# bioinfologics/w2rap-contigger

Hardware: AMD Instinct MI355X
Metric: step2_k60_canonical_kmers_per_s (higher is better)
Workload: dtype u64

## Files before the change

w2rap_contigger_amd/csrc/ctx.h:

```cpp
#pragma once
#include <hip/hip_runtime.h>
#include <stdint.h>
#include <stdio.h>
#include <stdlib.h>
#include <cstdlib>
#include <string>
#include <utility>
#include <vector>
#include "../../include/w2rap_step2.h"
#include "common.h"

namespace w2 {

struct Ctx;
}
struct w2rap_step2_ctx;
namespace w2 {
struct Ctx {
    int device = 0;
    hipStream_t stream = nullptr;
    hipStream_t stream2 = nullptr;
    unsigned long long* h_pinned = nullptr;
    std::string err;
    int sm_count = 256;

    uint64_t n = 0;
    const uint8_t* d_bases = nullptr;
    const uint64_t* d_boff = nullptr;
    const uint32_t* d_len = nullptr;
    const uint8_t* d_quals = nullptr;
    const uint64_t* d_qoff = nullptr;
    uint32_t max_len = 0;
    std::vector<void*> owned_reads;

    uint16_t* d_good = nullptr;
    uint32_t min_qual = 7, min_freq = 4;

    uint64_t M = 0, D = 0, S = 0;
    uint64_t hist[101] = {0};
    uint32_t NB = 0;
    uint32_t* d_bcount = nullptr;
    unsigned long long part_kmers[64] = {0};
    uint64_t* d_bbase = nullptr;
    uint32_t* d_recs = nullptr;
    uint64_t nrec = 0;
    uint64_t solid_cap = 0;
    uint64_t* d_shi = nullptr;
    uint64_t* d_slo = nullptr;
    uint32_t* d_scc = nullptr;
    Slot* d_table = nullptr;
    uint64_t tcap = 0;
    unsigned long long* d_filter32 = nullptr;
    uint64_t f32words = 0;
    uint8_t* d_sctx = nullptr;
    void* d_nbr = nullptr;
    bool wide_ids = false;
    uint64_t* d_chunk_start = nullptr;
    uint32_t* d_chunk_cnt = nullptr;
    uint64_t nchunks = 0;
    KRec* d_srec = nullptr;
    bool use_index = false;
    uint4* d_index = nullptr;
    uint64_t index_cap = 0, index_entries = 0;
    uint4* d_xindex = nullptr; uint64_t xindex_cap = 0, xindex_kmers = 0;
    bool index_prebuilt = false, bits_ready = false, filter_prebuilt = false;
    unsigned cs_ns = 0;
    unsigned cs_planned = 0;
    uint32_t cs_nbl = 0, cs_nseg = 0; const uint32_t* cs_recs = nullptr;
    bool cs_short_first = false;
    hipEvent_t cs_ev[16] = {};
    unsigned long long* cs_cnt = nullptr;
    uint64_t* cs_off = nullptr;
    uint32_t cs_chunk_cap = 0;
    uint8_t* d_unres = nullptr;
    bool fused_prune = false;
    std::vector<std::pair<uint64_t, uint64_t>> unfused_chunks;
    uint32_t* cs_defer = nullptr;
    uint64_t* g_hi = nullptr; uint64_t* g_lo = nullptr; uint32_t* g_cc = nullptr;
    uint64_t* g_cstart = nullptr; uint32_t* g_ccnt = nullptr;
    uint64_t g_cap = 0, g_n = 0, g_ccap = 0, g_nc = 0;
    bool g_open = false;
    hipEvent_t g_copied = nullptr;
    bool quality_done = false, counted = false, graphed = false, pathed_done = false;
    bool table_built = false;

    uint64_t E = 0;
    uint64_t rank_ends = 0;
    uint32_t* d_edge_nk = nullptr;
    uint64_t* d_edge_off = nullptr;
    uint8_t* d_edge_codes = nullptr;
    uint8_t* d_edge_bits = nullptr;
    uint64_t edge_bases = 0;
    uint64_t NO = 0, NV = 0;
    int32_t* d_fwdX = nullptr;
    int32_t* d_revX = nullptr;
    uint32_t* d_obj_edge = nullptr;
    ObjRec* d_otab = nullptr;
    int32_t* d_left = nullptr;
    int32_t* d_right = nullptr;
    uint64_t* d_from_off = nullptr;
    int32_t* d_from_v = nullptr;
    int32_t* d_from_e = nullptr;
    uint64_t* d_to_off = nullptr;
    int32_t* d_to_v = nullptr;
    int32_t* d_to_e = nullptr;
    int32_t* d_path_offset = nullptr;
    uint64_t* d_path_off = nullptr;
    int32_t* d_path_edges = nullptr;
    uint64_t path_total = 0;
    uint64_t n_pathed = 0, n_multipathed = 0;
    float ms_count = 0, ms_graph = 0, ms_path = 0;

    uint64_t ld_done = 0;
    void* shard = nullptr;
    std::vector<void*> owned;
    void* pump = nullptr;
    const uint32_t* d_qmask = nullptr;
    int qmask_min_qual = -1;
    int hint_min_qual = -1;
    bool hint_graph_only = false;
    bool quals_absent = false;
    uint8_t* d_qring = nullptr;
    void* pump2 = nullptr;
    hipStream_t copy_stream = nullptr;
    void* quals_job = nullptr;
    void* mask_job = nullptr; void* h_mask = nullptr; size_t h_mask_bytes = 0;
    uint32_t n_passes = 0;
// ... 254 lines not shown
```

w2rap_contigger_amd/csrc/step2_count.hip:

```cpp
#include <algorithm>
#include <chrono>
#include <cstdlib>
#include <cstring>
#include <type_traits>
#include "ctx.h"

namespace w2 {

constexpr unsigned QSLOTS = 256;
template <bool MASK>
__global__ void __launch_bounds__(256) k_good_len(uint64_t n, const uint8_t* __restrict__ quals, const uint32_t* __restrict__ qmask,
                                                   const uint64_t* __restrict__ qoff, const uint32_t* __restrict__ len,
                                                   uint32_t min_qual, uint16_t* __restrict__ good,
                                                   unsigned long long* __restrict__ total_kmers,
                                                   uint32_t* __restrict__ max_len) {
    constexpr unsigned CH = 4096;
    __shared__ __attribute__((aligned(16))) uint16_t gbits[CH + 16];
    __shared__ unsigned long long s_sum[4];
    __shared__ uint32_t s_max[4];
    const uint64_t r0 = (uint64_t)blockIdx.x * blockDim.x;
    const uint64_t r = r0 + threadIdx.x;
    const uint64_t rend = r0 + blockDim.x < n ? r0 + blockDim.x : n;
    const uint64_t base0 = qoff[r0], endo = qoff[rend];
    const unsigned shift = MASK ? (unsigned)(base0 & 31) : (unsigned)((reinterpret_cast<uintptr_t>(quals) + base0) & 15);
// ... 2232 lines not shown
}
int local_dict_slice(Ctx& c, uint64_t n_solid, uint64_t expected_total) {
    if (!c.stream2) return 0;
    if (!c.table_built) {
        if (c.d_table) { c.release(c.d_table); c.d_table = nullptr; }
        W2_TRY(table_alloc(c, std::max<uint64_t>(expected_total, n_solid), c.stream2));
        c.table_built = true; c.ld_done = 0;
    }
    if (n_solid > c.solid_cap) n_solid = c.solid_cap;
    if (n_solid > c.ld_done && 10 * c.tcap >= 13 * n_solid) {
        LAUNCH_ON(c, c.stream2, "k_table_insert", k_table_insert, dim3((unsigned)((n_solid - c.ld_done + 255) / 256)), dim3(256), 0, c.ld_done, n_solid,
                  c.d_shi, c.d_slo, c.d_table, c.tcap - 1);
        W2_HIP(hipGetLastError());
        c.ld_done = n_solid;
    }
    return 0;
}
int prune_local_chunks64(Ctx& c, uint8_t* sctx, uint64_t* nbr, uint8_t* unres) {
    hipStream_t st = c.stream;
    W2_HIP(hipMemsetAsync(unres, 0xFF, c.S, st));
    W2_HIP(hipMemsetAsync(sctx, 0xFF, c.S, st));
    if (!c.nchunks || getenv("W2RAP_NO_LOCAL_PRUNE")) return 0;
    const unsigned gl = (unsigned)std::min<uint64_t>(c.nchunks, (uint64_t)c.sm_count * 64);
    PL_LAUNCH(c, uint64_t, gl, c.S, c.nchunks, c.d_chunk_start, c.d_chunk_cnt, c.d_shi, c.d_slo, c.d_scc, sctx, nbr, unres);
    W2_HIP(hipGetLastError());
    return 0;
}
int prune_local_chunks32(Ctx& c, uint8_t* sctx, uint32_t* nbr, uint8_t* unres) {
    hipStream_t st = c.stream;
    W2_HIP(hipMemsetAsync(unres, 0xFF, c.S, st));
    W2_HIP(hipMemsetAsync(sctx, 0xFF, c.S, st));
    if (!c.nchunks || getenv("W2RAP_NO_LOCAL_PRUNE")) return 0;
    const unsigned gl = (unsigned)std::min<uint64_t>(c.nchunks, (uint64_t)c.sm_count * 64);
    PL_LAUNCH(c, uint32_t, gl, c.S, c.nchunks, c.d_chunk_start, c.d_chunk_cnt, c.d_shi, c.d_slo, c.d_scc, sctx, nbr, unres);
    W2_HIP(hipGetLastError());
    return 0;
}

template <class Id>
static int count_table_t(Ctx& c) {
    hipStream_t st = c.stream;
    if (!c.table_built) W2_TRY(table_alloc(c, c.S, st));
    const bool fused = c.fused_prune && sizeof(Id) == 4 && c.d_sctx && c.d_nbr && c.d_unres;
    Id* nbr = nullptr;
    if (fused) nbr = reinterpret_cast<Id*>(c.d_nbr);
    else {
        for (void* p : {(void*)c.d_sctx, (void*)c.d_nbr, (void*)c.d_unres}) if (p) c.release(p);
        c.d_unres = nullptr;
        W2_ALLOC(c.d_sctx, uint8_t, c.S);
        W2_ALLOC(nbr, Id, 2 * c.S);
        c.d_nbr = nbr;
    }
    c.fused_prune = false;
    if (c.S) {
        unsigned g = (unsigned)((c.S + 255) / 256);
        if (!c.table_built) {
            LAUNCH(c, "k_table_insert", k_table_insert, dim3(g), dim3(256), 0, (uint64_t)0, c.S, c.d_shi, c.d_slo, c.d_table, c.tcap - 1);
            W2_HIP(hipGetLastError());
        }
        uint8_t* d_unres = nullptr;
        if (fused) {
            d_unres = c.d_unres; c.d_unres = nullptr;
            for (auto& rg : c.unfused_chunks) {
                const uint64_t nch = rg.second - rg.first;
                if (!nch) continue;
                const unsigned gl = (unsigned)std::min<uint64_t>(nch, (uint64_t)c.sm_count * 64);
                PL_LAUNCH(c, Id, gl, c.S, nch, c.d_chunk_start + rg.first, c.d_chunk_cnt + rg.first, c.d_shi, c.d_slo, c.d_scc, c.d_sctx, nbr, d_unres);
                W2_HIP(hipGetLastError());
            }
        } else if (c.nchunks) {
            W2_ALLOC(d_unres, uint8_t, c.S);
            W2_HIP(hipMemsetAsync(d_unres, 0xFF, c.S, st));
            W2_HIP(hipMemsetAsync(c.d_sctx, 0xFF, c.S, st));
            const unsigned gl = (unsigned)std::min<uint64_t>(c.nchunks, (uint64_t)c.sm_count * 64);
            PL_LAUNCH(c, Id, gl, c.S, c.nchunks, c.d_chunk_start, c.d_chunk_cnt, c.d_shi, c.d_slo, c.d_scc, c.d_sctx, nbr, d_unres);
            W2_HIP(hipGetLastError());
        }
        if (c.table_built && c.stream2) {
            hipEvent_t ev;
            W2_HIP(hipEventCreateWithFlags(&ev, hipEventDisableTiming));
            W2_HIP(hipEventRecord(ev, c.stream2));
            W2_HIP(hipStreamWaitEvent(st, ev, 0));
            (void)hipEventDestroy(ev);
        }
        LAUNCH(c, "k_prune", k_prune<Id>, dim3(g), dim3(256), 0, (uint64_t)0, c.S, c.d_shi, c.d_slo, c.d_scc, c.d_table, c.tcap - 1, c.d_sctx, nbr,
               (const uint8_t*)d_unres);
        W2_HIP(hipGetLastError());
        W2_HIP(hipStreamSynchronize(st));
        if (d_unres) c.release(d_unres);
    }
    W2_HIP(hipStreamSynchronize(st));
    if (c.stream2) W2_HIP(hipStreamSynchronize(c.stream2));
    c.table_built = false;
    c.counted = true;
    return 0;
}
int count_table(Ctx& c) {
    if (c.S >= MAX_SOLID_KMERS) { c.err = "more than 2^32 solid k-mers on one GPU"; return W2RAP_E_LIMIT; }
    const char* wv = getenv("W2RAP_WIDE_IDS");
    c.wide_ids = c.S >= (1ull << 31) - 1 || (wv && atoi(wv) != 0);
    return c.wide_ids ? count_table_t<uint64_t>(c) : count_table_t<uint32_t>(c);
}

static unsigned auto_passes(uint64_t M) {
    size_t free_b = 0, total_b = 0;
    if (hipMemGetInfo(&free_b, &total_b) != hipSuccess || !free_b) return 1;
    const double need = (double)M / 15.0 * REC_BYTES * 1.25;
    unsigned p = (unsigned)(need / ((double)free_b / 4.0)) + 1;
    return std::min(p, 64u);
}

int phase_count(Ctx& c, uint32_t min_qual, uint32_t min_freq) {
    const bool trace = getenv("W2RAP_TRACE") != nullptr;
    auto now = [] { return std::chrono::duration<double>(std::chrono::steady_clock::now().time_since_epoch()).count(); };
    double t0 = now();
    W2_TRY(count_quality(c, min_qual));
    double t1 = now();
    const char* bv = getenv("W2RAP_BATCHES");
    const char* pv = getenv("W2RAP_PASSES");
    unsigned P = pv ? (unsigned)atoi(pv) : c.n_passes;
    if (!P) P = auto_passes(c.M);
    const uint32_t NB = default_buckets(c.M, 1);
    if (P > NB) P = NB;
    if (P < 1) P = 1;
    c.npass = P;
    double t_part = 0, t_cnt = 0;
    for (unsigned p = 0; p < P; ++p) {
        const uint32_t lo = (uint32_t)((uint64_t)NB * p / P), hi = (uint32_t)((uint64_t)NB * (p + 1) / P);
        unsigned nseg = 1;
        c.pass = p;
        double a = now();
        W2_TRY(count_partition_batched(c, NB, bv ? (unsigned)atoi(bv) : 4, &nseg, lo, hi));
        double b = now();
        W2_TRY(count_buckets(c, min_freq, hi - lo, nseg, c.d_recs, c.d_bcount, c.M, P == 1));
        c.release(c.d_recs); c.d_recs = nullptr;
        t_part += b - a; t_cnt += now() - b;
    }
    c.pass = 0; c.npass = 1;
    double t3 = now();
    W2_TRY(count_table(c));
    double t4 = now();
    if (trace) fprintf(stderr, "[w2rap] count: quality %.1f ms, partition %.1f ms, buckets %.1f ms, table %.1f ms (%u pass%s)\n",
                       (t1 - t0) * 1e3, t_part * 1e3, t_cnt * 1e3, (t4 - t3) * 1e3, P, P == 1 ? "" : "es");
    return 0;
}

}
```

w2rap_contigger_amd/csrc/step2_graph.hip:

```cpp
#include <algorithm>
#include "ctx.h"

namespace w2 {

enum { GE_LOOKUP = 1, GE_OFFSET = 2, GE_HINT_MISS = 4, GE_HINT_DUP = 8, GE_ASSIGN = 16, GE_HINT_LEN = 32 };

template <class Id>
__device__ inline Kmer oriented(const uint64_t* shi, const uint64_t* slo, Id v) {
    Kmer k{shi[v >> 1], slo[v >> 1]};
    return (v & 1) ? kmer_rc(k) : k;
}

template <class Id>
__global__ void __launch_bounds__(256) k_links(uint64_t S, const uint64_t* __restrict__ shi, const uint64_t* __restrict__ slo,
                                                const uint8_t* __restrict__ sctx, Id* nbr_nxt0) {
    constexpr Id NONE = NodeId<Id>::NONE, PAL = NodeId<Id>::PAL;
    uint64_t i = (uint64_t)blockIdx.x * blockDim.x + threadIdx.x;
    if (i >= S) return;
    Kmer k{shi[i], slo[i]};
    Id n0 = NONE, n1 = NONE;
    if (!kmer_is_pal(k)) {
        const Id s = nbr_nxt0[2 * i], p = nbr_nxt0[2 * i + 1];
        if (s < PAL) {
            unsigned cj = sctx[s >> 1]; if (s & 1) cj = brev8(cj);
            if (popc4(cj >> 4) == 1) n0 = s;
        }
        if (p < PAL) {
            unsigned cj = sctx[p >> 1]; if (p & 1) cj = brev8(cj);
            if (popc4(cj & 15) == 1) n1 = p ^ (Id)1;
        }
    }
    nbr_nxt0[2 * i] = n0; nbr_nxt0[2 * i + 1] = n1;
}

constexpr unsigned RT_BUF = 3072;
template <class Id>
__global__ void __launch_bounds__(256) k_rank_tiles(uint64_t S, uint64_t nchunks, const uint64_t* __restrict__ cstart,
                                                     const uint32_t* __restrict__ ccnt, const Id* __restrict__ nxt0,
                                                     unsigned long long* __restrict__ w, uint32_t* __restrict__ own,
                                                     Id* __restrict__ spl, unsigned long long* __restrict__ counters, uint64_t spl_cap) {
    constexpr Id NONE = NodeId<Id>::NONE;
    __shared__ __attribute__((aligned(16))) Id s_nx[RT_NODES];
    __shared__ uint32_t s_w[RT_NODES];
    __shared__ Id s_buf[RT_BUF];
    __shared__ uint32_t s_nbuf, s_run;
    __shared__ unsigned long long s_base;
    const unsigned tid = threadIdx.x, lane = tid & 63;
    if (tid == 0) { s_nbuf = 0; s_run = 0; }
    unsigned long long covered = 0;
    uint32_t ends = 0;
    auto flush = [&]() {
        const uint32_t n = s_nbuf;
        if (tid == 0) s_base = n ? atomicAdd(&counters[0], (unsigned long long)n) : 0ull;
        __syncthreads();
        const unsigned long long gb = s_base;
        for (unsigned i = tid; i < n; i += 256) if (gb + i < spl_cap) spl[gb + i] = s_buf[i];
        __syncthreads();
        if (tid == 0) s_nbuf = 0;
        __syncthreads();
    };
    const uint64_t ntiles = cstart ? nchunks : (S + RT - 1) / RT;
    for (uint64_t ch = blockIdx.x; ch < ntiles; ch += gridDim.x) {
        uint64_t c_start; uint32_t c_cnt;
        if (cstart) { c_start = cstart[ch]; c_cnt = ccnt[ch]; if (c_start + c_cnt > S) c_cnt = 0; }
        else { c_start = ch * RT; c_cnt = (uint32_t)(S - c_start < RT ? S - c_start : RT); }
        covered += c_cnt;
        for (uint32_t sub = 0; sub < c_cnt; sub += RT) {
            const uint64_t base = 2 * (c_start + sub);
            const uint32_t nloc = 2 * (c_cnt - sub < RT ? c_cnt - sub : RT);
            __syncthreads();
            {
                Id v4[4];
#pragma unroll
                for (unsigned q = 0; q < 4; ++q) v4[q] = 256 * q + tid < nloc ? nxt0[base + 256 * q + tid] : NONE;
#pragma unroll
                for (unsigned q = 0; q < 4; ++q) s_nx[256 * q + tid] = v4[q];
            }
            __syncthreads();
            bool listed[4];
            uint32_t mine = 0;
#pragma unroll
            for (unsigned q = 0; q < 4; ++q) {
                const unsigned x = 256 * q + tid;
                const Id nx = s_nx[x], px = s_nx[x ^ 1];
                const bool inside = px != NONE && (uint64_t)px - base < (uint64_t)nloc;
                const bool split = x < nloc && (nx == NONE || !inside);
                ends += x < nloc && nx == NONE;
                listed[q] = split && nx != NONE;
                mine += listed[q];
                s_w[x] = (split || x >= nloc) ? (0x80000000u | x) : ((1u << 10) | (uint32_t)(((uint64_t)px ^ 1ull) - base));
            }
            __syncthreads();
            for (unsigned round = 0; round < 11; ++round) {
                bool open = false;
#pragma unroll
                for (unsigned q = 0; q < 4; ++q) {
                    const unsigned x = 256 * q + tid;
                    uint32_t wx = s_w[x];
                    if (!(wx >> 31)) {
                        const uint32_t wp = s_w[wx & 1023u];
                        uint32_t steps = ((wx >> 10) & 0xFFFFFu) + ((wp >> 10) & 0xFFFFFu);
                        if (steps > 0xFFFFFu) steps = 0xFFFFFu;
                        wx = (wp & 0x800003FFu) | (steps << 10);
                        s_w[x] = wx;
                        open |= !(wx >> 31);
                    }
                }
                if (!__syncthreads_or(open)) break;
            }
            for (int d = 32; d > 0; d >>= 1) mine += __shfl_down(mine, d);
            if (lane == 0 && mine) atomicAdd(&s_run, mine);
            __syncthreads();
            if (s_nbuf + s_run > RT_BUF) flush();
            const uint32_t lbase = s_nbuf;
            __syncthreads();
            if (tid == 0) { s_nbuf = lbase + s_run; s_run = 0; }
#pragma unroll
            for (unsigned q = 0; q < 4; ++q) {
                const unsigned x = 256 * q + tid;
                if (x < nloc) {
                    const uint32_t wx = s_w[x]; const Id nx = s_nx[x];
                    const bool done = wx >> 31;
                    const uint32_t o = wx & 1023u, j = (wx >> 10) & 0xFFFFFu;
                    own[base + x] = done ? ((j << 12) | (x + RT_NODES - o)) : OWN_CIRCLE;
                    if (done) {
                        if (nx == NONE) w[base + x] = RankW<Id>::pack(0, (Id)(base + x));
                        else {
                            const uint64_t rel = (uint64_t)nx - base;
                            const bool next_split = rel >= (uint64_t)nloc || (s_w[rel] & 0xBFFFFFFFu) == (0x80000000u | (uint32_t)rel);
                            if (next_split) w[base + o] = RankW<Id>::pack(j + 1, nx);
// ... 978 lines not shown
    if (c.edge_bases > XPOS_MASK) return 0;
    unsigned long long* d_n = nullptr; uint32_t* d_f = nullptr;
    W2_ALLOC(d_n, unsigned long long, 128); W2_ALLOC(d_f, uint32_t, 4);
    W2_HIP(hipMemsetAsync(d_n, 0, 128 * 8, st));
    W2_HIP(hipMemsetAsync(d_f, 0, 16, st));
    unsigned run_max = 1u << 20;
    if (const char* v = getenv("W2RAP_TEST_INDEX_RUN_MAX")) { if (test_hook("W2RAP_TEST_INDEX_RUN_MAX")) run_max = (unsigned)std::max(1, atoi(v)); }
    LAUNCH(c, "k_index_mark", k_index_mark, dim3(grid_for(c.index_cap)), dim3(256), 0, c.index_cap, c.d_index, c.index_cap - 1, d_n, d_f, run_max);
    unsigned long long h_n[128];
    uint32_t h_run[4] = {0, 0, 0, 0};
    W2_HIP(hipMemcpyAsync(h_n, d_n, sizeof(h_n), hipMemcpyDeviceToHost, st));
    W2_HIP(hipMemcpyAsync(h_run, d_f, 16, hipMemcpyDeviceToHost, st));
    W2_HIP(hipStreamSynchronize(st));
    W2_HIP(hipGetLastError());
    if (h_run[1]) { c.release(d_n); c.release(d_f); c.err = "pathing index: a run of occupied slots longer than the marking pass walks (a degenerate key distribution)"; return W2RAP_E_LIMIT; }
    uint64_t hard = 0;
    for (unsigned i = 0; i < 64; ++i) hard += h_n[i];
    if (hard) {
        uint64_t cap = 1024;
        while (cap < hard * 24) cap <<= 1;
        if (test_hook("W2RAP_TEST_EXACT_SMALL")) cap = 1024;
        for (int attempt = 0;; ++attempt) {
            W2_ALLOC(c.d_xindex, uint4, cap);
            W2_HIP(hipMemsetAsync(c.d_xindex, 0xFF, cap * sizeof(uint4), st));
            W2_HIP(hipMemsetAsync(d_f, 0, 16, st));
            W2_HIP(hipMemsetAsync(d_n + 64, 0, 64 * 8, st));
            LAUNCH(c, "k_exact_insert", k_exact_insert, dim3(grid_for(c.index_cap)), dim3(256), 0, c.index_cap, (const uint4*)c.d_index, c.d_xindex, cap - 1, (const uint8_t*)c.d_edge_bits,
                   (const uint64_t*)c.d_edge_off, (const uint32_t*)c.d_edge_nk, d_f, d_n + 64);
            uint32_t h_f[4] = {0, 0, 0, 0};
            W2_HIP(hipMemcpyAsync(h_f, d_f, 16, hipMemcpyDeviceToHost, st));
            W2_HIP(hipMemcpyAsync(h_n, d_n, sizeof(h_n), hipMemcpyDeviceToHost, st));
            W2_HIP(hipStreamSynchronize(st));
            W2_HIP(hipGetLastError());
            uint64_t nin = 0;
            for (unsigned i = 64; i < 128; ++i) nin += h_n[i];
            if (!h_f[0] && 2 * nin <= cap) { c.xindex_cap = cap; c.xindex_kmers = nin; break; }
            if (attempt >= 24) { c.err = "pathing index: the exact table's sizing failed"; return W2RAP_E_LIMIT; }
            c.release(c.d_xindex); c.d_xindex = nullptr;
            cap <<= 2;
            while (cap < 2 * nin) cap <<= 1;
        }
    }
    if (getenv("W2RAP_TRACE")) fprintf(stderr, "[w2rap] pathing index: %llu entries of keys with more than %u entries, %llu k-mers around them in the exact table (%llu slots)\n",
                                       (unsigned long long)hard, IDX_HARD, (unsigned long long)c.xindex_kmers, (unsigned long long)c.xindex_cap);
    c.release(d_n); c.release(d_f);
    return 0;
}
int index_probe_all(Ctx& c, int32_t* d_edge, uint32_t* d_off) {
    if (c.S) LAUNCH(c, "k_index_probe", k_index_probe, dim3(grid_for(c.S)), dim3(256), 0, c.S, c.d_shi, c.d_slo, edge_index(c), d_edge, d_off);
    W2_HIP(hipGetLastError());
    return 0;
}

template <class Id>
static int run_ranking_t(Ctx& c, uint64_t N, const Id* nxt0, Id* nxt, uint32_t* rnk, unsigned long long* w, uint32_t* own, uint8_t* cyc, uint8_t* mid,
                         uint32_t* d_flags, const uint64_t* shi, const uint64_t* slo, bool use_chunks) {
    hipStream_t st = c.stream;
    unsigned long long* d_cnt = nullptr; Id* spl = nullptr;
    const uint64_t S = N / 2;
    uint64_t spl_cap = sizeof(Id) == 4 ? N : N / 4 + 4096;
    if (const char* v = getenv("W2RAP_SPL_CAP")) spl_cap = (uint64_t)atoll(v);
    W2_ALLOC(spl, Id, spl_cap); W2_ALLOC(d_cnt, unsigned long long, 4);
    unsigned long long h_cnt[4] = {0, 0, 0, 0};
    bool chunks = use_chunks && c.nchunks != 0 && !getenv("W2RAP_NO_RANK_CHUNKS");
    for (;;) {
        const uint64_t ntiles = chunks ? c.nchunks : (S + RT - 1) / RT;
        W2_HIP(hipMemsetAsync(d_cnt, 0, 32, st));
        LAUNCH(c, "k_rank_tiles", k_rank_tiles<Id>, dim3((unsigned)std::min<uint64_t>(ntiles ? ntiles : 1, (uint64_t)c.sm_count * 64)), dim3(256), 0,
               S, chunks ? c.nchunks : 0, chunks ? c.d_chunk_start : (const uint64_t*)nullptr, chunks ? c.d_chunk_cnt : (const uint32_t*)nullptr,
               nxt0, w, own, spl, d_cnt, spl_cap);
        W2_HIP(hipMemcpyAsync(h_cnt, d_cnt, 32, hipMemcpyDeviceToHost, st));
        W2_HIP(hipStreamSynchronize(st));
        if (h_cnt[1] != S) {
            if (!chunks) { c.err = "list ranking: tiles do not cover the k-mers"; return W2RAP_E_GRAPH; }
            chunks = false;
            continue;
        }
        if (h_cnt[0] <= spl_cap) break;
        c.release(spl);
        spl_cap = h_cnt[0] + 4096;
        W2_ALLOC(spl, Id, spl_cap);
    }
    const unsigned long long nspl = h_cnt[0];
    c.rank_ends = h_cnt[2];
    if (getenv("W2RAP_TRACE")) fprintf(stderr, "[w2rap] list ranking: %llu nodes, %llu listed splitters (%s tiles, %u-bit ids)\n", (unsigned long long)N, nspl, chunks ? "chunk" : "plain", (unsigned)(8 * sizeof(Id)));
    int rounds = 0;
    {
        const char* hv = getenv("W2RAP_RANK_HIER");
        if ((hv ? atoi(hv) != 0 : nspl >= (1u << 16)) && nspl) {
            const uint64_t sup_cap = nspl / 8 + 4096;
            Id* sup = nullptr; unsigned long long* d_ns = nullptr; unsigned long long ns = 0;
            W2_ALLOC(sup, Id, sup_cap); W2_ALLOC(d_ns, unsigned long long, 1);
            W2_HIP(hipMemsetAsync(d_ns, 0, 8, st));
            LAUNCH(c, "k_split_supers", k_split_supers<Id>, dim3((unsigned)((nspl + 256 * SUPERS_PER_THREAD - 1) / (256 * SUPERS_PER_THREAD))), dim3(256), 0, (uint64_t)nspl, spl, sup, d_ns, sup_cap);
            W2_HIP(hipMemcpyAsync(&ns, d_ns, 8, hipMemcpyDeviceToHost, st));
            W2_HIP(hipStreamSynchronize(st));
            if (ns && ns <= sup_cap) {
                unsigned long long* w0 = nullptr;
                W2_ALLOC(w0, unsigned long long, ns);
                LAUNCH(c, "k_split_walk", k_split_walk1<Id>, dim3(grid_for(ns)), dim3(256), 0, (uint64_t)ns, (const Id*)sup, w, w0);
                for (int round = 0; round < 2; ++round) {
                    LAUNCH(c, "k_split_super_jump", k_split_jump_super<Id>, dim3(grid_for(ns)), dim3(256), 0, (uint64_t)ns, (const Id*)sup, w, d_flags);
                    ++rounds;
                }
                LAUNCH(c, "k_split_walk", k_split_walk2<Id>, dim3(grid_for(ns)), dim3(256), 0, (uint64_t)ns, (const Id*)sup, w, (const unsigned long long*)w0);
                c.release(w0);
            }
            c.release(sup); c.release(d_ns);
        }
    }
    for (int round = 0; round < 40 && nspl; ++round) {
        W2_HIP(hipMemsetAsync(d_flags, 0, 4, st));
        LAUNCH(c, "k_split_jump", k_split_jump<Id>, dim3(grid_for(nspl)), dim3(256), 0, (uint64_t)nspl, spl, w, d_flags);
        uint32_t changed = 0;
        W2_HIP(hipMemcpyAsync(&changed, d_flags, 4, hipMemcpyDeviceToHost, st));
        W2_HIP(hipStreamSynchronize(st));
        ++rounds;
        if (!changed) break;
    }
    if (getenv("W2RAP_TRACE")) fprintf(stderr, "[w2rap] list ranking: %d jump launches\n", rounds);
    c.release(spl); c.release(d_cnt);
    if (mid) W2_HIP(hipMemsetAsync(mid, 0, N, st));
    LAUNCH(c, "k_rank_finish", k_rank_finish<Id>, dim3(grid_for(S)), dim3(256), 0, S, w, own, nxt0, shi, slo, nxt, rnk, cyc, mid, d_flags);
    W2_HIP(hipStreamSynchronize(st));
    return 0;
}
int run_ranking(Ctx& c, uint64_t N, const uint32_t* nxt0, uint32_t* nxt, uint32_t* rnk, unsigned long long* w, uint8_t* cyc, uint8_t* mid,
                uint32_t* d_flags, const uint64_t* shi, const uint64_t* slo, bool use_chunks) {
    uint32_t* own = nullptr;
    W2_ALLOC(own, uint32_t, N);
    const int rc = run_ranking_t<uint32_t>(c, N, nxt0, nxt, rnk, w, own, cyc, mid, d_flags, shi, slo, use_chunks);
    c.release(own);
    return rc;
}

static int graph_error(Ctx& c, uint32_t f) {
    if (f & GE_LOOKUP) { c.err = "neighbour k-mer lookup failed (ForceAssert, BuildReadQGraph.cc:265)"; return W2RAP_E_GRAPH; }
    if (f & GE_OFFSET) { c.err = "unipath longer than 16,777,215 k-mers (ForceAssertLe, ReadPather.h:122)"; return W2RAP_E_GRAPH; }
    if (f & GE_ASSIGN) { c.err = "k-mer left without an edge (BuildReadQGraph.cc:303)"; return W2RAP_E_GRAPH; }
    if (f & GE_HINT_MISS) { c.err = "edge_order_hint: a hinted edge is not a unipath of this graph"; return W2RAP_E_HINT; }
    if (f & GE_HINT_DUP) { c.err = "edge_order_hint: an edge is listed twice"; return W2RAP_E_HINT; }
    if (f & GE_HINT_LEN) { c.err = "edge_order_hint: a hinted edge has the wrong length"; return W2RAP_E_HINT; }
    return 0;
}

template <class Id>
static int rank_resolve_t(Ctx& c, uint64_t N, Id* nxt0, unsigned long long* rankw, uint32_t* own, uint8_t* cyc, uint8_t* mid, uint32_t* d_flags,
                          const uint64_t* shi, const uint64_t* slo, bool with_mid, bool* had_circles = nullptr) {
    hipStream_t st = c.stream;
    const uint64_t S = N / 2;
    uint32_t h_flags[4] = {0, 0, 0, 0};
    W2_TRY(run_ranking_t<Id>(c, N, nxt0, (Id*)nullptr, (uint32_t*)nullptr, rankw, own, cyc, mid, d_flags, with_mid ? shi : nullptr, slo, true));
    W2_HIP(hipMemcpyAsync(h_flags, d_flags, 16, hipMemcpyDeviceToHost, st));
    W2_HIP(hipStreamSynchronize(st));
    W2_TRY(graph_error(c, h_flags[1]));
    if (had_circles) *had_circles = h_flags[2] != 0;
    if (h_flags[2]) {
        Id *nx, *mn, *nx2, *mn2;
        W2_ALLOC(nx, Id, N); W2_ALLOC(mn, Id, N); W2_ALLOC(nx2, Id, N); W2_ALLOC(mn2, Id, N);
        LAUNCH(c, "k_minjump_init", k_minjump_init<Id>, dim3(grid_for(S)), dim3(256), 0, S, nxt0, cyc, nx, mn);
        for (int round = 0; round < 33; ++round) {
            LAUNCH(c, "k_minjump", k_minjump<Id>, dim3(grid_for(S)), dim3(256), 0, S, shi, slo, nx, mn, nx2, mn2);
            std::swap(nx, nx2); std::swap(mn, mn2);
        }
        LAUNCH(c, "k_cycle_cut", k_cycle_cut<Id>, dim3(grid_for(S)), dim3(256), 0, S, cyc, mn, nxt0);
        W2_HIP(hipStreamSynchronize(st));
        c.release(nx); c.release(mn); c.release(nx2); c.release(mn2);
        W2_HIP(hipMemsetAsync(d_flags, 0, 32, st));
        W2_TRY(run_ranking_t<Id>(c, N, nxt0, (Id*)nullptr, (uint32_t*)nullptr, rankw, own, cyc, mid, d_flags, with_mid ? shi : nullptr, slo, true));
        W2_HIP(hipMemcpyAsync(h_flags, d_flags, 16, hipMemcpyDeviceToHost, st));
        W2_HIP(hipStreamSynchronize(st));
        if (h_flags[2]) { c.err = "failed to close circle (BuildReadQGraph.cc:141)"; return W2RAP_E_GRAPH; }
    }
    return 0;
}
int rank_resolve32(Ctx& c, uint64_t N, uint32_t* nxt0, unsigned long long* rankw, uint32_t* own, uint8_t* cyc, uint8_t* mid, uint32_t* d_flags,
                   const uint64_t* shi, const uint64_t* slo, bool* had_circles) {
    return rank_resolve_t<uint32_t>(c, N, nxt0, rankw, own, cyc, mid, d_flags, shi, slo, false, had_circles);
}
int rank_resolve64(Ctx& c, uint64_t N, uint64_t* nxt0, unsigned long long* rankw, uint32_t* own, uint8_t* cyc, uint8_t* mid, uint32_t* d_flags,
                   const uint64_t* shi, const uint64_t* slo, bool* had_circles) {
    return rank_resolve_t<uint64_t>(c, N, nxt0, rankw, own, cyc, mid, d_flags, shi, slo, false, had_circles);
}

int graph_finish(Ctx& c) {
    hipStream_t st = c.stream;
    const uint64_t E = c.E;
    uint32_t* d_flags = nullptr;
    W2_ALLOC(d_flags, uint32_t, 8);
    W2_HIP(hipMemsetAsync(d_flags, 0, 32, st));
    uint32_t h_flags[4] = {0, 0, 0, 0};
    if (!c.bits_ready) {
        const uint64_t nby = (c.edge_bases + 3) / 4;
        W2_ALLOC(c.d_edge_bits, uint8_t, nby + 16);
        W2_HIP(hipMemsetAsync(c.d_edge_bits + nby, 0, 16, st));
        if (nby) LAUNCH(c, "k_pack_codes", k_pack_codes, dim3(grid_for(nby)), dim3(256), 0, nby, c.edge_bases, c.d_edge_codes, c.d_edge_bits);
    }
    c.bits_ready = false;
    if (c.use_index && c.d_table) { c.release(c.d_table); c.d_table = nullptr; }
    if (c.use_index && !c.index_prebuilt) W2_TRY(build_index(c));
    c.index_prebuilt = false;
    if (c.filter_prebuilt) c.filter_prebuilt = false;
    else {
    if (c.d_filter32) { c.release(c.d_filter32); c.d_filter32 = nullptr; }
    c.f32words = 0;
// ... 56 lines not shown
            break;
        }
        c.NV = nflag + 1;
        LAUNCH(c, "k_end_vertices", k_end_vertices, dim3(grid_for(NE)), dim3(256), 0, NE, eperm, eflag, excl, c.d_left, c.d_right);
    }
    const uint64_t NV = c.NV;
    W2_ALLOC(c.d_from_off, uint64_t, NV + 1); W2_ALLOC(c.d_to_off, uint64_t, NV + 1);
    W2_ALLOC(c.d_from_v, int32_t, NO); W2_ALLOC(c.d_from_e, int32_t, NO);
    W2_ALLOC(c.d_to_v, int32_t, NO); W2_ALLOC(c.d_to_e, int32_t, NO);
    uint32_t* deg = nullptr; uint64_t* akeys = nullptr; uint32_t* avals = nullptr;
    W2_ALLOC(deg, uint32_t, NV); W2_ALLOC(akeys, uint64_t, NO); W2_ALLOC(avals, uint32_t, NO);
    for (int dir = 0; dir < 2; ++dir) {
        const int32_t* a = dir == 0 ? c.d_left : c.d_right;
        const int32_t* b = dir == 0 ? c.d_right : c.d_left;
        W2_HIP(hipMemsetAsync(deg, 0, (NV ? NV : 1) * 4, st));
        if (NO) {
            LAUNCH(c, "k_adj_keys", k_adj_keys, dim3(grid_for(NO)), dim3(256), 0, NO, a, b, akeys, avals, deg);
            W2_TRY(sort_pairs_u64(c, akeys, avals, NO, 0, 64));
            LAUNCH(c, "k_adj_out", k_adj_out, dim3(grid_for(NO)), dim3(256), 0, NO, avals, b, dir == 0 ? c.d_from_v : c.d_to_v,
                               dir == 0 ? c.d_from_e : c.d_to_e);
        }
        W2_TRY(exclusive_scan_u32_to_u64(c, deg, dir == 0 ? c.d_from_off : c.d_to_off, NV));
    }
    if (c.d_otab) { c.release(c.d_otab); c.d_otab = nullptr; }
    W2_ALLOC(c.d_otab, ObjRec, NO);
    if (NO) LAUNCH(c, "k_obj_table", k_obj_table, dim3(grid_for(NO)), dim3(256), 0, NO, c.d_obj_edge, c.d_edge_nk, c.d_edge_off, c.d_edge_codes,
                   c.d_right, c.d_from_off, c.d_from_e, c.d_otab);
    W2_HIP(hipStreamSynchronize(st));
    if (c.stream2) W2_HIP(hipStreamSynchronize(c.stream2));
    W2_HIP(hipGetLastError());
    for (void* p : {(void*)d_nobj, (void*)d_ooff, (void*)ehash, (void*)ehi, (void*)elo, (void*)ktmp, (void*)excl,
                    (void*)eperm, (void*)eflag, (void*)deg, (void*)akeys, (void*)avals, (void*)d_flags})
        c.release(p);
    c.graphed = true;
    return 0;
}

template <class Id>
static int phase_graph_t(Ctx& c, const w2rap_edge_hint* hint) {
    constexpr Id NONE = NodeId<Id>::NONE; (void)NONE;
    hipStream_t st = c.stream;
    const uint64_t S = c.S, N = 2 * S;
    const uint64_t mask = c.tcap - 1;
    uint32_t* d_flags = nullptr;
    W2_ALLOC(d_flags, uint32_t, 8);
    W2_HIP(hipMemsetAsync(d_flags, 0, 32, st));
    Id* nxt0 = reinterpret_cast<Id*>(c.d_nbr);
    unsigned long long* rankw = nullptr; uint32_t* own = nullptr;
    W2_ALLOC(rankw, unsigned long long, N); W2_ALLOC(own, uint32_t, N);
    uint8_t *cyc = nullptr, *mid = nullptr, *is_head = nullptr;
    W2_ALLOC(cyc, uint8_t, N); W2_ALLOC(mid, uint8_t, N);
    uint32_t h_flags[4] = {0, 0, 0, 0};
    if (S) {
        LAUNCH(c, "k_links", k_links<Id>, dim3(grid_for(S)), dim3(256), 0, S, c.d_shi, c.d_slo, c.d_sctx, nxt0);
        W2_TRY(rank_resolve_t<Id>(c, N, nxt0, rankw, own, cyc, mid, d_flags, c.d_shi, c.d_slo, true));
    }
    c.release(cyc); cyc = nullptr;
    unsigned long long* d_nheads = nullptr;
    W2_ALLOC(d_nheads, unsigned long long, 1);
    W2_HIP(hipMemsetAsync(d_nheads, 0, 8, st));
    const uint64_t head_cap = S ? c.rank_ends + 1 : 1;
    Id *head_v, *edge_head; uint32_t* perm;
    uint64_t *key_hi, *key_lo, *key_tmp;
    W2_ALLOC(is_head, uint8_t, N);
    W2_ALLOC(head_v, Id, head_cap); W2_ALLOC(key_hi, uint64_t, head_cap); W2_ALLOC(key_lo, uint64_t, head_cap);
    if (S) LAUNCH(c, "k_heads", k_heads<Id>, dim3((unsigned)((S + 256 * HEADS_PER - 1) / (256 * HEADS_PER))), dim3(256), 0, S, c.d_shi, c.d_slo, nxt0, own, rankw, mid, is_head,
                              head_v, key_hi, key_lo, d_nheads, head_cap, d_flags, hint == nullptr);
    W2_HIP(hipGetLastError());
    unsigned long long E = 0;
    W2_HIP(hipMemcpyAsync(&E, d_nheads, 8, hipMemcpyDeviceToHost, st));
    W2_HIP(hipMemcpyAsync(h_flags, d_flags, 16, hipMemcpyDeviceToHost, st));
    W2_HIP(hipStreamSynchronize(st));
    W2_TRY(graph_error(c, h_flags[1]));
    if (E > head_cap) { c.err = "more canonical heads than chain ends"; return W2RAP_E_GRAPH; }
    if (E >= (1ull << 31)) { c.err = "more than 2^31 unipaths (edge ids are int, paths/long/ReadPath.h)"; return W2RAP_E_LIMIT; }
    c.E = E;
    c.release(c.d_nbr); c.d_nbr = nullptr; nxt0 = nullptr;
    c.release(mid); mid = nullptr;
    W2_ALLOC(perm, uint32_t, E); W2_ALLOC(edge_head, Id, E);
    W2_ALLOC(key_tmp, uint64_t, E);
    W2_ALLOC(c.d_edge_nk, uint32_t, E);
    if (hint) {
        if (hint->n_edges != E) {
            c.err = "edge_order_hint has " + std::to_string(hint->n_edges) + " edges, the graph has " + std::to_string(E);
            return W2RAP_E_HINT;
        }
        std::vector<uint64_t> hh(E), hl(E);
        for (uint64_t e = 0; e < E; ++e) {
            if (hint->len[e] < K) { c.err = "edge_order_hint: edge shorter than K"; return W2RAP_E_HINT; }
            const uint8_t* p = hint->packed + hint->byte_off[e];
            uint64_t hi = 0, lo = 0;
            for (unsigned t = 0; t < 30; ++t) hi = (hi << 2) | ((p[t >> 2] >> (2 * (t & 3))) & 3);
            for (unsigned t = 30; t < 60; ++t) lo = (lo << 2) | ((p[t >> 2] >> (2 * (t & 3))) & 3);
            hh[e] = hi; hl[e] = lo;
        }
        uint32_t* d_hlen = nullptr;
        W2_ALLOC(d_hlen, uint32_t, E);
        W2_HIP(hipMemcpyAsync(key_hi, hh.data(), E * 8, hipMemcpyHostToDevice, st));
        W2_HIP(hipMemcpyAsync(key_lo, hl.data(), E * 8, hipMemcpyHostToDevice, st));
        W2_HIP(hipMemcpyAsync(d_hlen, hint->len, E * 4, hipMemcpyHostToDevice, st));
        if (E) LAUNCH(c, "k_edge_from_hint", k_edge_from_hint<Id>, dim3(grid_for(E)), dim3(256), 0, E, key_hi, key_lo, d_hlen, c.d_table, mask, c.d_shi, c.d_slo, is_head,
                                  own, rankw, edge_head, c.d_edge_nk, d_flags);
        W2_HIP(hipMemcpyAsync(h_flags, d_flags, 16, hipMemcpyDeviceToHost, st));
        W2_HIP(hipStreamSynchronize(st));
        W2_TRY(graph_error(c, h_flags[1]));
        c.release(d_hlen);
    } else {
        if (E) {
// ... 53 lines not shown
```

Measured before the change: 40.80 billion.

## Fuse link resolution into tile list ranking and prefetch next tile

```diff
diff --git a/w2rap_contigger_amd/csrc/ctx.h b/w2rap_contigger_amd/csrc/ctx.h
--- a/w2rap_contigger_amd/csrc/ctx.h
+++ b/w2rap_contigger_amd/csrc/ctx.h
@@ -73,6 +73,8 @@
     uint64_t* cs_off = nullptr;
     uint32_t cs_chunk_cap = 0;
     uint8_t* d_unres = nullptr;
+    bool own_count = false;
+    bool tile_links_ok = false;
     bool fused_prune = false;
     std::vector<std::pair<uint64_t, uint64_t>> unfused_chunks;
     uint32_t* cs_defer = nullptr;
diff --git a/w2rap_contigger_amd/csrc/step2_count.hip b/w2rap_contigger_amd/csrc/step2_count.hip
--- a/w2rap_contigger_amd/csrc/step2_count.hip
+++ b/w2rap_contigger_amd/csrc/step2_count.hip
@@ -2308,6 +2308,8 @@
         c.d_nbr = nbr;
     }
     c.fused_prune = false;
+    c.tile_links_ok = !fused && sizeof(Id) == 4 && c.own_count && c.nchunks != 0 && !getenv("W2RAP_NO_LOCAL_PRUNE");
+    c.own_count = false;
     if (c.S) {
         unsigned g = (unsigned)((c.S + 255) / 256);
         if (!c.table_built) {
@@ -2321,7 +2323,7 @@
                 const uint64_t nch = rg.second - rg.first;
                 if (!nch) continue;
                 const unsigned gl = (unsigned)std::min<uint64_t>(nch, (uint64_t)c.sm_count * 64);
-                PL_LAUNCH(c, Id, gl, c.S, nch, c.d_chunk_start + rg.first, c.d_chunk_cnt + rg.first, c.d_shi, c.d_slo, c.d_scc, c.d_sctx, nbr, d_unres);
+                PL_LAUNCH(c, Id, gl, c.S / c.nchunks * nch, nch, c.d_chunk_start + rg.first, c.d_chunk_cnt + rg.first, c.d_shi, c.d_slo, c.d_scc, c.d_sctx, nbr, d_unres);
                 W2_HIP(hipGetLastError());
             }
         } else if (c.nchunks) {
@@ -2393,6 +2395,7 @@
         t_part += b - a; t_cnt += now() - b;
     }
     c.pass = 0; c.npass = 1;
+    c.own_count = P == 1;
     double t3 = now();
     W2_TRY(count_table(c));
     double t4 = now();
diff --git a/w2rap_contigger_amd/csrc/step2_graph.hip b/w2rap_contigger_amd/csrc/step2_graph.hip
--- a/w2rap_contigger_amd/csrc/step2_graph.hip
+++ b/w2rap_contigger_amd/csrc/step2_graph.hip
@@ -11,6 +11,12 @@
     return (v & 1) ? kmer_rc(k) : k;
 }
 
+template <class Id>
+__device__ inline Id link_rule(Id nb, unsigned port, unsigned cj) {
+    if (nb & 1) cj = brev8(cj);
+    if (port == 0) return popc4(cj >> 4) == 1 ? nb : NodeId<Id>::NONE;
+    return popc4(cj & 15) == 1 ? (Id)(nb ^ (Id)1) : NodeId<Id>::NONE;
+}
 template <class Id>
 __global__ void __launch_bounds__(256) k_links(uint64_t S, const uint64_t* __restrict__ shi, const uint64_t* __restrict__ slo,
                                                 const uint8_t* __restrict__ sctx, Id* nbr_nxt0) {
@@ -21,25 +27,19 @@
     Id n0 = NONE, n1 = NONE;
     if (!kmer_is_pal(k)) {
         const Id s = nbr_nxt0[2 * i], p = nbr_nxt0[2 * i + 1];
-        if (s < PAL) {
-            unsigned cj = sctx[s >> 1]; if (s & 1) cj = brev8(cj);
-            if (popc4(cj >> 4) == 1) n0 = s;
-        }
-        if (p < PAL) {
-            unsigned cj = sctx[p >> 1]; if (p & 1) cj = brev8(cj);
-            if (popc4(cj & 15) == 1) n1 = p ^ (Id)1;
-        }
+        if (s < PAL) n0 = link_rule<Id>(s, 0, sctx[s >> 1]);
+        if (p < PAL) n1 = link_rule<Id>(p, 1, sctx[p >> 1]);
     }
     nbr_nxt0[2 * i] = n0; nbr_nxt0[2 * i + 1] = n1;
 }
 
 constexpr unsigned RT_BUF = 3072;
-template <class Id>
-__global__ void __launch_bounds__(256) k_rank_tiles(uint64_t S, uint64_t nchunks, const uint64_t* __restrict__ cstart,
-                                                     const uint32_t* __restrict__ ccnt, const Id* __restrict__ nxt0,
+template <class Id, bool LINKS>
+__global__ void __launch_bounds__(256) __attribute__((amdgpu_waves_per_eu(sizeof(Id) == 4 ? 7 : 4))) k_rank_tiles(uint64_t S, uint64_t nchunks, const uint64_t* __restrict__ cstart,
+                                                     const uint32_t* __restrict__ ccnt, Id* __restrict__ nxt0, const uint8_t* __restrict__ sctx,
                                                      unsigned long long* __restrict__ w, uint32_t* __restrict__ own,
                                                      Id* __restrict__ spl, unsigned long long* __restrict__ counters, uint64_t spl_cap) {
-    constexpr Id NONE = NodeId<Id>::NONE;
+    constexpr Id NONE = NodeId<Id>::NONE, PAL = NodeId<Id>::PAL; (void)PAL;
     __shared__ __attribute__((aligned(16))) Id s_nx[RT_NODES];
     __shared__ uint32_t s_w[RT_NODES];
     __shared__ Id s_buf[RT_BUF];
@@ -60,22 +60,59 @@
         __syncthreads();
     };
     const uint64_t ntiles = cstart ? nchunks : (S + RT - 1) / RT;
+    auto load_desc = [&](uint64_t ch, uint64_t& st_, uint32_t& cn_) {
+        st_ = 0; cn_ = 0;
+        if (ch >= ntiles) return;
+        if (cstart) { st_ = cstart[ch]; cn_ = ccnt[ch]; if (st_ + cn_ > S) cn_ = 0; }
+        else { st_ = ch * RT; cn_ = (uint32_t)(S - st_ < RT ? S - st_ : RT); }
+    };
+    auto load_tile = [&](uint64_t k0, uint32_t nk, Id (&v_)[4], uint32_t& b_) {
+        if (nk > RT) nk = RT;
+#pragma unroll
+        for (unsigned q = 0; q < 4; ++q) v_[q] = 256 * q + tid < 2 * nk ? nxt0[2 * k0 + 256 * q + tid] : NONE;
+        if (LINKS) b_ = (tid < nk ? (uint32_t)sctx[k0 + tid] : 0u) | (256 + tid < nk ? (uint32_t)sctx[k0 + 256 + tid] << 8 : 0u);
+    };
+    uint64_t st_c, st_n; uint32_t cn_c, cn_n;
+    Id nv[4]; uint32_t nb = 0;
+    load_desc(blockIdx.x, st_c, cn_c);
+    load_tile(st_c, cn_c, nv, nb);
+    load_desc((uint64_t)blockIdx.x + gridDim.x, st_n, cn_n);
     for (uint64_t ch = blockIdx.x; ch < ntiles; ch += gridDim.x) {
-        uint64_t c_start; uint32_t c_cnt;
-        if (cstart) { c_start = cstart[ch]; c_cnt = ccnt[ch]; if (c_start + c_cnt > S) c_cnt = 0; }
-        else { c_start = ch * RT; c_cnt = (uint32_t)(S - c_start < RT ? S - c_start : RT); }
+        const uint64_t c_start = st_c; const uint32_t c_cnt = cn_c;
+        Id v4[4]; uint32_t cb = nb;
+#pragma unroll
+        for (unsigned q = 0; q < 4; ++q) v4[q] = nv[q];
+        st_c = st_n; cn_c = cn_n;
+        load_tile(st_c, cn_c, nv, nb);
+        load_desc(ch + 2 * (uint64_t)gridDim.x, st_n, cn_n);
         covered += c_cnt;
         for (uint32_t sub = 0; sub < c_cnt; sub += RT) {
             const uint64_t base = 2 * (c_start + sub);
             const uint32_t nloc = 2 * (c_cnt - sub < RT ? c_cnt - sub : RT);
+            if (sub) load_tile(c_start + sub, c_cnt - sub, v4, cb);
             __syncthreads();
-            {
-                Id v4[4];
-#pragma unroll
-                for (unsigned q = 0; q < 4; ++q) v4[q] = 256 * q + tid < nloc ? nxt0[base + 256 * q + tid] : NONE;
-#pragma unroll
-                for (unsigned q = 0; q < 4; ++q) s_nx[256 * q + tid] = v4[q];
+            if (LINKS) {
+                uint8_t* s_cx = reinterpret_cast<uint8_t*>(s_w);
+                s_cx[tid] = (uint8_t)cb; s_cx[256 + tid] = (uint8_t)(cb >> 8);
+                __syncthreads();
+#pragma unroll
+                for (unsigned q = 0; q < 4; ++q) {
+                    const unsigned x = 256 * q + tid;
+                    const Id n = v4[q], other = __shfl_xor(n, 1);
+                    if (x < nloc) {
+                        Id l = NONE;
+                        if (n < PAL && other != (Id)(n ^ (Id)1)) {
+                            const uint64_t rel = (uint64_t)(n >> 1) - (c_start + sub);
+                            const unsigned cj = rel < (uint64_t)(nloc >> 1) ? s_cx[rel] : sctx[n >> 1];
+                            l = link_rule<Id>(n, x & 1u, cj);
+                        }
+                        v4[q] = l;
+                        nxt0[base + x] = l;
+                    }
+                }
             }
+#pragma unroll
+            for (unsigned q = 0; q < 4; ++q) s_nx[256 * q + tid] = v4[q];
             __syncthreads();
             bool listed[4];
             uint32_t mine = 0;
@@ -1160,9 +1197,20 @@
     return 0;
 }
 
-template <class Id>
-static int run_ranking_t(Ctx& c, uint64_t N, const Id* nxt0, Id* nxt, uint32_t* rnk, unsigned long long* w, uint32_t* own, uint8_t* cyc, uint8_t* mid,
-                         uint32_t* d_flags, const uint64_t* shi, const uint64_t* slo, bool use_chunks) {
+__global__ void __launch_bounds__(256) k_chunk_cover(uint64_t S, uint64_t nchunks, const uint64_t* __restrict__ cstart, const uint32_t* __restrict__ ccnt,
+                                                      unsigned long long* __restrict__ covered) {
+    unsigned long long n = 0; unsigned big = 0;
+    for (uint64_t ch = (uint64_t)blockIdx.x * blockDim.x + threadIdx.x; ch < nchunks; ch += (uint64_t)gridDim.x * blockDim.x) {
+        const uint64_t st = cstart[ch]; const uint32_t cn = ccnt[ch];
+        if (st + cn <= S) { n += cn; big += cn > RT; }
+    }
+    for (int d = 32; d > 0; d >>= 1) { n += __shfl_down(n, d); big += __shfl_down(big, d); }
+    if ((threadIdx.x & 63) == 0 && n) atomicAdd(covered, n);
+    if ((threadIdx.x & 63) == 0 && big) atomicAdd(covered + 1, (unsigned long long)big);
+}
+template <class Id>
+static int run_ranking_t(Ctx& c, uint64_t N, Id* nxt0, Id* nxt, uint32_t* rnk, unsigned long long* w, uint32_t* own, uint8_t* cyc, uint8_t* mid,
+                         uint32_t* d_flags, const uint64_t* shi, const uint64_t* slo, bool use_chunks, const uint8_t* link_ctx = nullptr) {
     hipStream_t st = c.stream;
     unsigned long long* d_cnt = nullptr; Id* spl = nullptr;
     const uint64_t S = N / 2;
@@ -1171,16 +1219,32 @@
     W2_ALLOC(spl, Id, spl_cap); W2_ALLOC(d_cnt, unsigned long long, 4);
     unsigned long long h_cnt[4] = {0, 0, 0, 0};
     bool chunks = use_chunks && c.nchunks != 0 && !getenv("W2RAP_NO_RANK_CHUNKS");
+    if (link_ctx && chunks) {
+        W2_HIP(hipMemsetAsync(d_cnt, 0, 32, st));
+        LAUNCH(c, "k_chunk_cover", k_chunk_cover, dim3((unsigned)std::min<uint64_t>(grid_for(c.nchunks), 256)), dim3(256), 0, S, c.nchunks, (const uint64_t*)c.d_chunk_start, (const uint32_t*)c.d_chunk_cnt, d_cnt);
+        W2_HIP(hipMemcpyAsync(h_cnt, d_cnt, 16, hipMemcpyDeviceToHost, st));
+        W2_HIP(hipStreamSynchronize(st));
+        if (getenv("W2RAP_TRACE")) fprintf(stderr, "[w2rap] list ranking: the chunk list covers %llu of %llu k-mers, %llu chunks of several tiles\n", h_cnt[0], (unsigned long long)S, h_cnt[1]);
+        if (h_cnt[0] != S) chunks = false;
+    }
     for (;;) {
         const uint64_t ntiles = chunks ? c.nchunks : (S + RT - 1) / RT;
+        const dim3 grid((unsigned)std::min<uint64_t>(ntiles ? ntiles : 1, (uint64_t)c.sm_count * 64));
         W2_HIP(hipMemsetAsync(d_cnt, 0, 32, st));
-        LAUNCH(c, "k_rank_tiles", k_rank_tiles<Id>, dim3((unsigned)std::min<uint64_t>(ntiles ? ntiles : 1, (uint64_t)c.sm_count * 64)), dim3(256), 0,
-               S, chunks ? c.nchunks : 0, chunks ? c.d_chunk_start : (const uint64_t*)nullptr, chunks ? c.d_chunk_cnt : (const uint32_t*)nullptr,
-               nxt0, w, own, spl, d_cnt, spl_cap);
+        if (link_ctx)
+            LAUNCH(c, "k_rank_tiles", (k_rank_tiles<Id, true>), grid, dim3(256), 0,
+                   S, chunks ? c.nchunks : 0, chunks ? c.d_chunk_start : (const uint64_t*)nullptr, chunks ? c.d_chunk_cnt : (const uint32_t*)nullptr,
+                   nxt0, link_ctx, w, own, spl, d_cnt, spl_cap);
+        else
+            LAUNCH(c, "k_rank_tiles", (k_rank_tiles<Id, false>), grid, dim3(256), 0,
+                   S, chunks ? c.nchunks : 0, chunks ? c.d_chunk_start : (const uint64_t*)nullptr, chunks ? c.d_chunk_cnt : (const uint32_t*)nullptr,
+                   nxt0, (const uint8_t*)nullptr, w, own, spl, d_cnt, spl_cap);
+        const bool converted = link_ctx != nullptr;
+        link_ctx = nullptr;
         W2_HIP(hipMemcpyAsync(h_cnt, d_cnt, 32, hipMemcpyDeviceToHost, st));
         W2_HIP(hipStreamSynchronize(st));
         if (h_cnt[1] != S) {
-            if (!chunks) { c.err = "list ranking: tiles do not cover the k-mers"; return W2RAP_E_GRAPH; }
+            if (!chunks || converted) { c.err = "list ranking: tiles do not cover the k-mers"; return W2RAP_E_GRAPH; }
             chunks = false;
             continue;
         }
@@ -1237,7 +1301,7 @@
                 uint32_t* d_flags, const uint64_t* shi, const uint64_t* slo, bool use_chunks) {
     uint32_t* own = nullptr;
     W2_ALLOC(own, uint32_t, N);
-    const int rc = run_ranking_t<uint32_t>(c, N, nxt0, nxt, rnk, w, own, cyc, mid, d_flags, shi, slo, use_chunks);
+    const int rc = run_ranking_t<uint32_t>(c, N, const_cast<uint32_t*>(nxt0), nxt, rnk, w, own, cyc, mid, d_flags, shi, slo, use_chunks);
     c.release(own);
     return rc;
 }
@@ -1254,11 +1318,11 @@
 
 template <class Id>
 static int rank_resolve_t(Ctx& c, uint64_t N, Id* nxt0, unsigned long long* rankw, uint32_t* own, uint8_t* cyc, uint8_t* mid, uint32_t* d_flags,
-                          const uint64_t* shi, const uint64_t* slo, bool with_mid, bool* had_circles = nullptr) {
+                          const uint64_t* shi, const uint64_t* slo, bool with_mid, bool* had_circles = nullptr, const uint8_t* link_ctx = nullptr) {
     hipStream_t st = c.stream;
     const uint64_t S = N / 2;
     uint32_t h_flags[4] = {0, 0, 0, 0};
-    W2_TRY(run_ranking_t<Id>(c, N, nxt0, (Id*)nullptr, (uint32_t*)nullptr, rankw, own, cyc, mid, d_flags, with_mid ? shi : nullptr, slo, true));
+    W2_TRY(run_ranking_t<Id>(c, N, nxt0, (Id*)nullptr, (uint32_t*)nullptr, rankw, own, cyc, mid, d_flags, with_mid ? shi : nullptr, slo, true, link_ctx));
     W2_HIP(hipMemcpyAsync(h_flags, d_flags, 16, hipMemcpyDeviceToHost, st));
     W2_HIP(hipStreamSynchronize(st));
     W2_TRY(graph_error(c, h_flags[1]));
@@ -1421,8 +1485,11 @@
     W2_ALLOC(cyc, uint8_t, N); W2_ALLOC(mid, uint8_t, N);
     uint32_t h_flags[4] = {0, 0, 0, 0};
     if (S) {
-        LAUNCH(c, "k_links", k_links<Id>, dim3(grid_for(S)), dim3(256), 0, S, c.d_shi, c.d_slo, c.d_sctx, nxt0);
-        W2_TRY(rank_resolve_t<Id>(c, N, nxt0, rankw, own, cyc, mid, d_flags, c.d_shi, c.d_slo, true));
+        const char* tv = getenv("W2RAP_TILE_LINKS");
+        const bool tile_links = c.tile_links_ok && sizeof(Id) == 4 && tv && atoi(tv) != 0;
+        if (getenv("W2RAP_TRACE")) fprintf(stderr, "[w2rap] links: %s\n", tile_links ? "inside the tile ranking" : "k_links");
+        if (!tile_links) LAUNCH(c, "k_links", k_links<Id>, dim3(grid_for(S)), dim3(256), 0, S, c.d_shi, c.d_slo, c.d_sctx, nxt0);
+        W2_TRY(rank_resolve_t<Id>(c, N, nxt0, rankw, own, cyc, mid, d_flags, c.d_shi, c.d_slo, true, nullptr, tile_links ? (const uint8_t*)c.d_sctx : nullptr));
     }
     c.release(cyc); cyc = nullptr;
     unsigned long long* d_nheads = nullptr;
```

After: 40.79 billion. Within noise of the previous version (-0.0%).
